# ishine/dmel_codec

Hardware: AMD Instinct MI355X
Metric: audio-sec/sec (encode+decode RTF) @24 kHz batch 32 (higher is better)
Workload: dtype f32; 1 GPU; cfg2: encode+decode, 24000 Hz, 80 mel, 8 FSQ groups [7, 5, 5], WaveNet 20+20 layers, BigVGAN-base, batch 32 x 1 s per GPU; lanes=3, vocoder_streams=1

## Files before the change

### dmel_codec_amd/_lib.py

```python
from __future__ import annotations

import ctypes as C
import os
from typing import Optional, Sequence

import torch

_HERE = os.path.dirname(os.path.abspath(__file__))
LIB_PATH = os.environ.get("DMEL_LIB") or os.path.join(_HERE, "libdmel_hip.so")
_lib: Optional[C.CDLL] = None

i64p = C.POINTER(C.c_int64)
i32p = C.POINTER(C.c_int32)
f32p = C.POINTER(C.c_float)
vp = C.c_void_p
GRAD_READY_FN = C.CFUNCTYPE(None, vp, C.c_int64, C.c_int64)


class BigVGANConfig(C.Structure):
    _fields_ = [
        ("num_mels", C.c_int),
        ("upsample_initial_channel", C.c_int),
        ("num_upsamples", C.c_int),
        ("upsample_rates", C.c_int * 8),
# ... 10 lines not shown


PROTOTYPES = {
    "dmel_last_error": (C.c_char_p, []),
    "dmel_abi_version": (C.c_int, []),
    "dmel_stft_plan_create": (C.c_int, [C.POINTER(vp), C.c_int, C.c_int, C.c_int, C.c_int, C.c_int, C.c_double, C.c_double, vp]),
    "dmel_stft_plan_destroy": (None, [vp]),
    "dmel_mel_basis_host": (C.c_int, [C.c_int, C.c_int, C.c_int, C.c_double, C.c_double, vp]),
    "dmel_stft_plan_mel_basis": (C.c_int, [vp, vp]),
    "dmel_stft_num_frames": (C.c_int64, [vp, C.c_int64]),
    "dmel_stft_logmel_f32": (C.c_int, [vp, vp, C.c_int64, vp, vp, C.c_int, C.c_int64, vp]),
    "dmel_resample_f32": (C.c_int, [vp, vp, vp, C.c_int, C.c_int64, C.c_int64, C.c_int, C.c_int, C.c_int, vp]),
    "dmel_resample_window_f32": (C.c_int, [vp, C.c_int64, C.c_int64, C.c_int64, vp, vp, C.c_int, C.c_int64, C.c_int64, C.c_int64, C.c_int, C.c_int,
                                           C.c_int, vp]),
    "dmel_resample_window_items_f32": (C.c_int, [vp, C.c_int64, C.c_int64, i64p, i64p, vp, C.c_int64, i64p, vp, C.c_int64, i64p, C.c_int, i64p,
                                                 C.c_int, i64p, i64p, i64p, vp, vp]),
    "dmel_pcm_convert_items": (C.c_int, [C.POINTER(vp), i32p, C.POINTER(vp), i32p, i64p, C.c_int, vp, vp]),
    "dmel_pcm_convert_items_ch": (C.c_int, [C.POINTER(vp), i32p, i32p, i32p, C.POINTER(vp), i32p, i32p, i64p, C.c_int, vp, vp]),
    "dmel_stft_f32": (C.c_int, [vp, vp, C.c_int64, vp, vp, vp, C.c_int, C.c_int64, vp]),
    "dmel_stft_window_f32": (C.c_int, [vp, vp, C.c_int64, C.c_int64, C.c_int64, vp, vp, vp, C.c_int, C.c_int64, C.c_int64, C.c_int64, vp]),
    "dmel_stft_window_items_f32": (C.c_int, [vp, vp, C.c_int64, C.c_int64, i64p, i64p, vp, vp, vp, C.c_int, i64p, i64p, i64p, vp, vp]),
    "dmel_aa_snake_f32": (C.c_int, [vp, vp, vp, vp, vp, vp, C.c_int, C.c_int, C.c_int, C.c_int64, vp]),
    "dmel_aa_snake_items_f32": (C.c_int, [vp, vp, vp, vp, vp, vp, C.c_int, C.c_int, C.c_int, C.c_int64, vp, vp]),
    "dmel_aa_snake_backward_f32": (C.c_int, [vp, vp, vp, vp, vp, vp, vp, vp, vp, C.c_int, C.c_int, C.c_int, C.c_int64, vp]),
    "dmel_discriminator_create": (C.c_int, [C.POINTER(vp)]),
    "dmel_discriminator_destroy": (None, [vp]),
    "dmel_discriminator_set_tensor": (C.c_int, [vp, C.c_char_p, vp, C.POINTER(C.c_int64), C.c_int]),
    "dmel_discriminator_finalize": (C.c_int, [vp]),
    "dmel_discriminator_out_frames": (C.c_int64, [vp, C.c_int64]),
    "dmel_discriminator_workspace_bytes": (C.c_size_t, [vp, C.c_int, C.c_int, C.c_int64]),
    "dmel_discriminator_forward": (C.c_int, [vp, vp, vp, C.c_int, C.c_int, C.c_int64, vp, C.c_size_t, vp]),
    "dmel_discriminator_enable_training": (C.c_int, [vp, C.c_int]),
    "dmel_discriminator_set_train_precision": (C.c_int, [vp, C.c_int]),
    "dmel_discriminator_refresh": (C.c_int, [vp, C.c_int, C.POINTER(C.c_char_p), C.POINTER(vp), vp]),
    "dmel_discriminator_train_workspace_bytes": (C.c_size_t, [vp, C.c_int, C.c_int, C.c_int64]),
    "dmel_discriminator_grad_floats": (C.c_int64, [vp]),
    "dmel_discriminator_grad_slot": (C.c_int, [vp, C.c_char_p, C.POINTER(C.c_int64), C.POINTER(C.c_int64)]),
    "dmel_discriminator_forward_train": (C.c_int, [vp, vp, vp, C.c_int, C.c_int, C.c_int64, vp, C.c_size_t, vp]),
    "dmel_discriminator_backward": (C.c_int, [vp, vp, vp, vp, C.c_int, C.c_int, C.c_int64, vp, C.c_size_t, vp]),
    "dmel_convnext_create": (C.c_int, [C.POINTER(vp), C.c_int]),
    "dmel_convnext_destroy": (None, [vp]),
    "dmel_convnext_set_tensor": (C.c_int, [vp, C.c_char_p, vp, C.POINTER(C.c_int64), C.c_int]),
    "dmel_convnext_enable_training": (C.c_int, [vp, C.c_int]),
    "dmel_convnext_set_train_precision": (C.c_int, [vp, C.c_int]),
    "dmel_convnext_finalize": (C.c_int, [vp]),
    "dmel_convnext_workspace_bytes": (C.c_size_t, [vp, C.c_int, C.c_int64]),
# ... 178 lines not shown
```

### dmel_codec_amd/csrc/aa_snake.hip

```cpp
#include "ops.h"
#include "snake_dev.h"

namespace dmel {

constexpr int kSnakeTile = 1024;
constexpr int kSnakeFwdTile = 1008;

typedef float f32x4 __attribute__((ext_vector_type(4)));

template <bool VEC>
__device__ __forceinline__ void aa_snake_row(const float* __restrict__ xr, float* __restrict__ yr, const float* __restrict__ alpha,
                                             const float* __restrict__ beta, const Taps12& tu, const Taps12& td, int logscale, int c, int T,
                                             int first, int nsub, float* xs, float* ve, float* vo) {
  float a = alpha[c], bt = beta ? beta[c] : a;
  if (logscale) {
    bt = beta ? expf(bt) : expf(a);
    a = expf(a);
  }
  const float inv_b = 1.0f / (bt + 1e-9f);
  const int tid = threadIdx.x;
  auto fetch = [&](int t0) {
    const int s = t0 - 8 + 4 * tid;
    if (VEC && s >= 0 && s + 4 <= T) return *reinterpret_cast<const f32x4*>(xr + s);
    f32x4 v;
    v.x = xr[min(max(s, 0), T - 1)];
    v.y = xr[min(max(s + 1, 0), T - 1)];
    v.z = xr[min(max(s + 2, 0), T - 1)];
    v.w = xr[min(max(s + 3, 0), T - 1)];
    return v;
  };
  float aa[8], bb[8];
#pragma unroll
  for (int i = 0; i < 8; ++i) { aa[i] = a; bb[i] = inv_b; }
  f32x4 pre = {0.f, 0.f, 0.f, 0.f};
  if (first < T) pre = fetch(first);
  for (int sub = 0; sub < nsub; ++sub) {
    const int t0 = first + sub * kSnakeFwdTile;
    if (t0 >= T) break;
    const int len = min(kSnakeFwdTile, T - t0);
    if (sub) __syncthreads();
    *reinterpret_cast<f32x4*>(xs + 4 * tid) = pre;
    if (sub + 1 < nsub && t0 + kSnakeFwdTile < T) pre = fetch(t0 + kSnakeFwdTile);
    __syncthreads();
    if (4 * tid < len + 6) {
      float w[12];
      lds_read3_b128(xs + 4 * tid, w);
      float u[8];
#pragma unroll
      for (int i = 0; i < 4; ++i) {
        float ue = 0.f, uo = 0.f;
#pragma unroll
        for (int j = 0; j < 6; ++j) {
          ue = fmaf(tu.f[2 * j + 1], w[i + 7 - j], ue);
          uo = fmaf(tu.f[2 * j], w[i + 8 - j], uo);
        }
        u[2 * i] = ue;
        u[2 * i + 1] = uo;
      }
      snake_n(u, aa, bb);
      *reinterpret_cast<f32x4*>(ve + 4 * tid) = f32x4{u[0], u[2], u[4], u[6]};
      *reinterpret_cast<f32x4*>(vo + 4 * tid) = f32x4{u[1], u[3], u[5], u[7]};
    }
    __syncthreads();
    const int pe = T - t0 + 3;
    if (t0 == 0 || pe < len + 6) {
      if (tid < 3) {
        if (t0 == 0) ve[tid] = vo[tid] = ve[3];
        if (pe + tid < len + 6) ve[pe + tid] = vo[pe + tid] = vo[pe - 1];
      }
      __syncthreads();
    }
    if (4 * tid < len) {
      float e[12], o[12];
      lds_read3_b128(ve + 4 * tid, e);
      lds_read3_b128(vo + 4 * tid, o);
      f32x4 out;
#pragma unroll
      for (int i = 0; i < 4; ++i) {
        float acc = td.f[0] * o[i];
#pragma unroll
        for (int k = 1; k < 6; ++k) {
          acc = fmaf(td.f[2 * k - 1], e[i + k], acc);
          acc = fmaf(td.f[2 * k], o[i + k], acc);
        }
        out[i] = fmaf(td.f[11], e[i + 6], acc);
      }
      float* yp = yr + t0 + 4 * tid;
      if (VEC) {
        *reinterpret_cast<f32x4*>(yp) = out;
      } else {
#pragma unroll
        for (int i = 0; i < 4; ++i)
          if (4 * tid + i < len) yp[i] = out[i];
      }
    }
  }
}

template <bool VEC>
__global__ __launch_bounds__(256) void aa_snake_kernel(const float* __restrict__ x, float* __restrict__ y,
                                                          const float* __restrict__ alpha, const float* __restrict__ beta,
                                                          Taps12 tu, Taps12 td, int logscale, int C, int T, int nsub) {
  __shared__ __attribute__((aligned(16))) float xs[kSnakeFwdTile + 16];
  __shared__ __attribute__((aligned(16))) float ve[kSnakeFwdTile + 16];
  __shared__ __attribute__((aligned(16))) float vo[kSnakeFwdTile + 16];
  const int c = blockIdx.y, b = blockIdx.z;
  const int64_t row = ((int64_t)b * C + c) * T;
  aa_snake_row<VEC>(x + row, y + row, alpha, beta, tu, td, logscale, c, T, blockIdx.x * nsub * kSnakeFwdTile, nsub, xs, ve, vo);
}

__global__ __launch_bounds__(256) void aa_snake_items_kernel(const float* __restrict__ x, float* __restrict__ y,
                                                                const float* __restrict__ alpha, const float* __restrict__ beta,
                                                                Taps12 tu, Taps12 td, int logscale, int C, int T,
                                                                const int64_t* __restrict__ len, int nsub) {
  __shared__ __attribute__((aligned(16))) float xs[kSnakeFwdTile + 16];
  __shared__ __attribute__((aligned(16))) float ve[kSnakeFwdTile + 16];
  __shared__ __attribute__((aligned(16))) float vo[kSnakeFwdTile + 16];
  const int c = blockIdx.y, b = blockIdx.z;
  const int n = (int)min(max(len[b], (int64_t)0), (int64_t)T);
  const int first = blockIdx.x * nsub * kSnakeFwdTile;
  if (first >= n) return;
  const int64_t row = ((int64_t)b * C + c) * T;
  const float* xr = x + row;
  float* yr = y + row;
  const bool vec = n % 4 == 0 && (reinterpret_cast<uintptr_t>(xr) | reinterpret_cast<uintptr_t>(yr)) % 16 == 0;
  if (vec) aa_snake_row<true>(xr, yr, alpha, beta, tu, td, logscale, c, n, first, nsub, xs, ve, vo);
  else aa_snake_row<false>(xr, yr, alpha, beta, tu, td, logscale, c, n, first, nsub, xs, ve, vo);
}

template <bool PARAMS>
__global__ __launch_bounds__(256) void aa_snake_bwd_kernel(const float* __restrict__ x, const float* __restrict__ dy,
                                                            float* dx, const float* __restrict__ alpha,
                                                            const float* __restrict__ beta, float* __restrict__ dalpha,
                                                            float* __restrict__ dbeta, const float* __restrict__ radd, const float* racc,
                                                            Taps12 tu, Taps12 td, int logscale, int C, int T) {
  __shared__ float xs[kSnakeTile + 12];
  __shared__ float dys[kSnakeTile + 12];
  __shared__ float dvs[2 * (kSnakeTile + 6)];
  __shared__ float dxs[kSnakeTile];
  __shared__ float red[2][4];
  const int c = blockIdx.y, b = blockIdx.z, tid = threadIdx.x;
  const int t0 = blockIdx.x * kSnakeTile;
  const int len = min(kSnakeTile, T - t0);
  const float* xr = x + ((int64_t)b * C + c) * T;
  const float* dyr = dy + ((int64_t)b * C + c) * T;
  float* dxr = dx + ((int64_t)b * C + c) * T;
  float a = alpha[c], bt = beta ? beta[c] : a;
  if (logscale) {
    bt = beta ? expf(bt) : expf(a);
    a = expf(a);
// ... 167 lines not shown
    else hipLaunchKernelGGL(aa_snake_kernel<false>, grid, dim3(256), 0, s, x, y, alpha, beta, tu, td, logscale, C, (int)T, nsub);
  }
  DMEL_HIP(hipGetLastError());
  return DMEL_OK;
}

int launch_aa_snake_items(const float* x, float* y, const float* alpha, const float* beta, const float* up_taps_host,
                          const float* down_taps_host, int logscale, int B, int C, int64_t T, const int64_t* len, hipStream_t s) {
  DMEL_CHECK_ARG(x && y && alpha && up_taps_host && down_taps_host && len, "aa_snake_items: NULL argument");
  DMEL_CHECK_ARG(B > 0 && C > 0 && T > 0 && B <= 65535 && C <= 65535 && T < ((int64_t)1 << 30), "aa_snake_items: bad shape");
  Taps12 tu, td;
  for (int i = 0; i < 12; ++i) { tu.f[i] = 2.f * up_taps_host[i]; td.f[i] = down_taps_host[i]; }
  constexpr int nsub = 3;
  constexpr int span = kSnakeFwdTile * nsub;
  dim3 grid((unsigned)((T + span - 1) / span), (unsigned)C, (unsigned)B);
  {
    ProfScope ps("aa_snake", s, 0.0, 8.0 * (double)B * C * (double)T);
    hipLaunchKernelGGL(aa_snake_items_kernel, grid, dim3(256), 0, s, x, y, alpha, beta, tu, td, logscale, C, (int)T, len, nsub);
  }
  DMEL_HIP(hipGetLastError());
  return DMEL_OK;
}

}

extern "C" int dmel_aa_snake_items_f32(const float* x, float* y, const float* alpha, const float* beta, const float* up_filter12_host,
                                       const float* down_filter12_host, int logscale, int B, int C, int64_t T, const int64_t* lengths_dev,
                                       void* stream) {
  return dmel::launch_aa_snake_items(x, y, alpha, beta, up_filter12_host, down_filter12_host, logscale, B, C, T, lengths_dev,
                                     (hipStream_t)stream);
}

extern "C" int dmel_aa_snake_backward_f32(const float* x, const float* dy, float* dx, const float* alpha, const float* beta,
                                          float* dalpha, float* dbeta, const float* up_filter12_host, const float* down_filter12_host,
                                          int logscale, int B, int C, int64_t T, void* stream) {
  return dmel::launch_aa_snake_bwd(x, dy, dx, alpha, beta, dalpha, dbeta, up_filter12_host, down_filter12_host, logscale, B, C, T,
                                   (hipStream_t)stream);
}

extern "C" int dmel_aa_snake_backward_input_f32(const float* x, const float* dy, const float* add , float* dx, const float* alpha,
                                                const float* beta, const float* up_filter12_host, const float* down_filter12_host,
                                                int logscale, int B, int C, int64_t T, void* stream) {
  return dmel::launch_aa_snake_bwd_input(x, dy, dx, add, nullptr, alpha, beta, up_filter12_host, down_filter12_host, logscale, B, C, T,
                                         (hipStream_t)stream);
}

// ... 5 lines not shown
```

### dmel_codec_amd/csrc/modules.hip

```cpp
#include <cmath>
#include <cstdlib>
#include <map>
#include <memory>
#include <mutex>

#include "ops.h"

using namespace dmel;

namespace {

struct HostTensor {
  std::vector<float> v;
  std::vector<int64_t> shape;
  int64_t numel() const { return (int64_t)v.size(); }
};

struct TensorStore {
  std::map<std::string, HostTensor> t;
  int set(const char* key, const float* data, const int64_t* shape, int ndim) {
    DMEL_CHECK_ARG(key && data && shape && ndim >= 0 && ndim <= 4, "set_tensor: bad argument");
    HostTensor h;
    int64_t n = 1;
    for (int i = 0; i < ndim; ++i) { h.shape.push_back(shape[i]); n *= shape[i]; }
// ... 2572 lines not shown
  float* ua = bufs[4];

  {
    ConvRun r = run_1seg(mel, c.num_mels, T, x, c.upsample_initial_channel, T, B);
    r.seg[0].in_len = len_at(0);
    r.precision = prec;
    DMEL_TRY(launch_conv(m->conv_pre, r, st));
  }
  int64_t Tc = T;
  int ch = c.upsample_initial_channel;
  for (int i = 0; i < c.num_upsamples; ++i) {
    const UpStage& us = m->ups[i];
    const int64_t Tn = Tc * us.u;
    DMEL_TRY(launch_up_stage(us, x, xu, B, Tc, prec, st, len_at(i)));
    ch = us.Cout;
    Tc = Tn;
    const int64_t bs = (int64_t)ch * Tc;
    const bool multi = m->multi;
    const int64_t* len = len_at(i + 1);
    if (multi) {
      DMEL_HIP(hipEventRecord(m->ev_fork, st));
      for (int k = 0; k < dmel_bigvgan::kSide; ++k) DMEL_HIP(hipStreamWaitEvent(m->side[k], m->ev_fork, 0));
    }
    for (int j = 0; j < c.num_kernels; ++j) {
      const AmpBlock& ab = m->blocks[(size_t)i * c.num_kernels + j];
      hipStream_t sj = (multi && j > 0) ? m->side[j - 1] : st;
      float *xj = bufs[3 + 3 * j], *uj = bufs[4 + 3 * j], *vj = bufs[5 + 3 * j];
      const float* xin = xu;
      const char* fuse_env = getenv("DMEL_FUSE_SNAKE");
      const bool fuse = fuse_env && fuse_env[0] == '1' && !lengths;
      for (int l = 0; l < 3; ++l) {
        if (l == 0 && multi && j > 0) DMEL_HIP(hipStreamWaitEvent(sj, m->ev_stag[j - 1], 0));
        if (c.resblock_type == 2) {
          ConvRun r2 = run_1seg(uj, ch, Tc, l < 2 ? xj : xs, ch, Tc, B);
          r2.seg[0].in_len = len;
          r2.res = xin; r2.res_bs = bs; r2.res_cs = Tc;
          r2.precision = prec;
          const bool fuse2 = fuse && conv_snake_eligible(ab.c1[l], r2);
          if (!fuse2) DMEL_TRY(act(xin, uj, ab.act[l], ch, Tc, len, sj));
          if (!fuse2 && l == 0 && multi && j + 1 < c.num_kernels) DMEL_HIP(hipEventRecord(m->ev_stag[j], sj));
          if (l == 2) {
            r2.accumulate = j > 0;
            if (j == c.num_kernels - 1) r2.out_div = (float)c.num_kernels;
            if (multi && j > 0) DMEL_HIP(hipStreamWaitEvent(sj, m->ev_chain[j - 1], 0));
          }
          if (fuse2) {
            r2.seg[0].x = xin;
            DMEL_TRY(launch_conv_snake(ab.c1[l], r2, ab.act[l].alpha.as<float>(), ab.act[l].beta.as<float>(), m->taps_up, m->taps_dn, logscale, sj));
            if (l == 0 && multi && j + 1 < c.num_kernels) DMEL_HIP(hipEventRecord(m->ev_stag[j], sj));
          } else {
            DMEL_TRY(launch_conv(ab.c1[l], r2, sj));
          }
          if (l == 2 && multi && j + 1 < c.num_kernels) DMEL_HIP(hipEventRecord(m->ev_chain[j], sj));
          xin = xj;
          continue;
        }
        ConvRun r1 = run_1seg(uj, ch, Tc, vj, ch, Tc, B);
        r1.seg[0].in_len = len;
        r1.precision = prec;
        if (fuse && conv_snake_eligible(ab.c1[l], r1)) {
          r1.seg[0].x = xin;
          DMEL_TRY(launch_conv_snake(ab.c1[l], r1, ab.act[2 * l].alpha.as<float>(), ab.act[2 * l].beta.as<float>(), m->taps_up, m->taps_dn, logscale, sj));
          if (l == 0 && multi && j + 1 < c.num_kernels) DMEL_HIP(hipEventRecord(m->ev_stag[j], sj));
        } else {
          DMEL_TRY(act(xin, uj, ab.act[2 * l], ch, Tc, len, sj));
          if (l == 0 && multi && j + 1 < c.num_kernels) DMEL_HIP(hipEventRecord(m->ev_stag[j], sj));
          DMEL_TRY(launch_conv(ab.c1[l], r1, sj));
        }
        ConvRun r2 = run_1seg(uj, ch, Tc, l < 2 ? xj : xs, ch, Tc, B);
        r2.seg[0].in_len = len;
        r2.res = xin; r2.res_bs = bs; r2.res_cs = Tc;
        r2.precision = prec;
        const bool fuse2 = fuse && conv_snake_eligible(ab.c2[l], r2);
        if (!fuse2) DMEL_TRY(act(vj, uj, ab.act[2 * l + 1], ch, Tc, len, sj));
        if (l == 2) {
          r2.accumulate = j > 0;
          if (j == c.num_kernels - 1) r2.out_div = (float)c.num_kernels;
          if (multi && j > 0) DMEL_HIP(hipStreamWaitEvent(sj, m->ev_chain[j - 1], 0));
        }
        if (fuse2) {
          r2.seg[0].x = vj;
          DMEL_TRY(launch_conv_snake(ab.c2[l], r2, ab.act[2 * l + 1].alpha.as<float>(), ab.act[2 * l + 1].beta.as<float>(), m->taps_up, m->taps_dn, logscale, sj));
        } else {
          DMEL_TRY(launch_conv(ab.c2[l], r2, sj));
        }
        if (l == 2 && multi && j + 1 < c.num_kernels) DMEL_HIP(hipEventRecord(m->ev_chain[j], sj));
        xin = xj;
      }
    }
    if (multi) {
      for (int k = 0; k < dmel_bigvgan::kSide && k + 1 < c.num_kernels; ++k) {
        DMEL_HIP(hipEventRecord(m->ev_join[k], m->side[k]));
        DMEL_HIP(hipStreamWaitEvent(st, m->ev_join[k], 0));
      }
    }
    std::swap(x, xs);
  }
  const int64_t* len_out = len_at(c.num_upsamples);
  DMEL_TRY(act(x, ua, m->act_post, ch, Tc, len_out, st));
  return launch_conv_post(ua, audio, m->post_w.as<float>(), m->post_bias, c.use_tanh_at_final ? ACT_TANH : ACT_CLAMP1, B, ch, 7,
                          Tc, st, len_out);
}

extern "C" int dmel_bigvgan_forward(const dmel_bigvgan* m, const float* mel, float* audio, int B, int64_t T, void* workspace,
                                    size_t workspace_bytes, void* stream) {
  return bigvgan_forward_impl(m, mel, nullptr, audio, B, T, workspace, workspace_bytes, stream);
}

extern "C" int dmel_bigvgan_forward_items(const dmel_bigvgan* m, const float* mel, const int64_t* lengths_dev, float* audio, int B, int64_t T,
                                          void* workspace, size_t workspace_bytes, void* stream) {
  DMEL_CHECK_ARG(lengths_dev, "bigvgan_forward_items: NULL lengths");
  return bigvgan_forward_impl(m, mel, lengths_dev, audio, B, T, workspace, workspace_bytes, stream);
}

extern "C" int dmel_bigvgan_enable_input_grad(dmel_bigvgan* m, int on) {
  DMEL_CHECK_ARG(m, "bigvgan_enable_input_grad: NULL handle");
  if (!m->ready) { set_error("bigvgan_enable_input_grad: handle not finalized"); return DMEL_EMISSING; }
  const dmel_bigvgan_config& c = m->cfg;
  if (!on) {
    m->input_grad = false;
    m->conv_preT = PackedConv();
// ... 243 lines not shown
```

### dmel_codec_amd/csrc/ops.h

```cpp
#pragma once
#include "conv.h"

namespace dmel {

struct FsqConst {
  int n_levels;
  int levels[4], half_width[4], basis[4];
  float half_l[4], offset[4], shift[4];
  int prebound;
  int strict;
};

int make_fsq_const(FsqConst& k, const int* levels, int n, int prebound);
int launch_fsq_encode(const float* z, const float* w_in, const float* b_in, int32_t* ids, float* prequant,
                      const FsqConst& k, int B, int G, int C, int64_t T4, hipStream_t s, const int64_t* len = nullptr);
int launch_fsq_decode(const int32_t* ids, const float* w_out, const float* b_out, float* z, const FsqConst& k, int B,
                      int G, int C, int64_t T4, hipStream_t s, const int64_t* len = nullptr);
int launch_fsq_backward(const float* x, const float* dout, const float* w_in, const float* b_in, const float* w_out, float* dx,
                        float* dw_in, float* db_in, float* dw_out, float* db_out, float* scratch, const FsqConst& k, int B, int G, int C,
                        int64_t T4, hipStream_t s);
int launch_dwconv_ln(const float* x, float* y, const float* dw_w, const float* dw_b, const float* ln_w, const float* ln_b,
                     int N, int C, int64_t T, hipStream_t s, float* h0 = nullptr, const int64_t* len = nullptr, int len_div = 1);
int launch_conv_post(const float* x, float* y, const float* w_dev, float bias, int act, int B, int C, int K, int64_t T,
                     hipStream_t s, const int64_t* len = nullptr);
// ... 18 lines not shown
};
int launch_wavenet_fused(const WaveNetFused& f, const float* x, float* y, const int64_t* in_len, const int64_t* out_len, int len_div, int N,
                         int64_t T, hipStream_t st);
constexpr int kStreamMaxL = 32;
int launch_wavenet_stream(const WaveNetFused& f, const float* x, float* hist, float* skip, float* y, const int64_t* out_len, int len_div,
                          int N, int64_t cap, const int64_t* prev, const int64_t* next, hipStream_t st);
constexpr int kStreamRowInts(int L) { return 2 * (L + 1) + 1; }
int launch_wavenet_stream_items(const WaveNetFused& f, const float* x, float* hist, float* skip, float* y, const int64_t* out_len, int len_div,
                                int N, int64_t cap, const int64_t* prev, const int64_t* next, int32_t* tab_dev, hipStream_t st);
int launch_shift_lengths(const int64_t* len, int64_t shift, int64_t* out, int n, hipStream_t st);
int launch_copy_windows(const float* src, float* dst, int N, int C, int64_t cap, const int32_t* tab, int stride, int i_shift, int i_end,
                        int len_div, int64_t max_cols, int64_t cols_total, hipStream_t st);
int launch_shift_lengths_items(const int64_t* len, const int32_t* tab, int stride, int i_shift, int64_t* out, int n, hipStream_t st);
struct LenScales {
  static constexpr int kMax = 9;
  int64_t v[kMax];
};
int launch_length_tables(const int64_t* len, int64_t* tab, int n, int64_t T, int stages, const LenScales& scale, hipStream_t st);
int launch_stage_lengths(const int64_t* len, int64_t* tab, int n, int64_t T, int stages, int down, hipStream_t st);
int launch_aa_snake(const float* x, float* y, const float* alpha, const float* beta, const float* up_taps_host,
                    const float* down_taps_host, int logscale, int B, int C, int64_t T, hipStream_t s);
int launch_aa_snake_items(const float* x, float* y, const float* alpha, const float* beta, const float* up_taps_host,
                          const float* down_taps_host, int logscale, int B, int C, int64_t T, const int64_t* len, hipStream_t s);
int launch_aa_snake_bwd_input(const float* x, const float* dy, float* dx, const float* radd, const float* racc, const float* alpha,
                              const float* beta, const float* up_taps_host, const float* down_taps_host, int logscale, int B, int C,
                              int64_t T, hipStream_t s);

bool conv_snake_eligible(const PackedConv& pc, const ConvRun& r);
int launch_conv_snake(const PackedConv& pc, const ConvRun& r, const float* alpha, const float* beta, const float* up_taps_host,
                      const float* down_taps_host, int logscale, hipStream_t stream);

bool conv_pc_eligible(const PackedConv& pc, const ConvRun& r, bool any_size = false);
int launch_conv_pc(const PackedConv& pc, const ConvRun& r, hipStream_t stream);

int launch_gate_fwd(const float* pre, float* z, int N, int C, int64_t T, hipStream_t s);
int launch_gate_bwd(const float* dz, const float* pre, float* dpre, int N, int C, int64_t T, hipStream_t s);
int launch_resskip_fwd(const float* x, const float* o, float* xn, float* skipsum, int first, int N, int C, int64_t T, hipStream_t s);
int launch_resskip_bwd(const float* gx, const float* gs, float* go, float* gxs, int N, int C, int64_t T, hipStream_t s);
int launch_silu_fwd(const float* u, float* y, int64_t total, hipStream_t s);
int launch_silu_bwd(const float* g, const float* u, float* du, int64_t total, hipStream_t s);
int launch_scale(const float* x, float* y, float k, int64_t total, hipStream_t s);
int launch_gelu_fwd(const float* u, float* g, int64_t total, hipStream_t s);
int launch_gelu_bwd(const float* dg, const float* u, float* du, int64_t total, hipStream_t s);
int launch_layerscale_res_fwd(const float* x, const float* v, const float* gamma, float* y, int N, int C, int64_t T, hipStream_t s);
int launch_layerscale_bwd(const float* dy, const float* v, const float* gamma, float* dv, float* dgamma, int N, int C, int64_t T,
                          hipStream_t s);
// ... 13 lines not shown
```

### include/dmel_hip.h

```cpp
#ifndef DMEL_HIP_H
#define DMEL_HIP_H

#include <stddef.h>
#include <stdint.h>

#ifdef __cplusplus
extern "C" {
#endif

#define DMEL_OK 0
#define DMEL_EINVAL (-1)
#define DMEL_EUNSUPPORTED (-2)
#define DMEL_EMISSING (-3)

#define DMEL_PRECISION_FP32 0
#define DMEL_PRECISION_BF16 1
#define DMEL_PRECISION_FP32_MFMA 2
#define DMEL_PRECISION_FP32_F16X2 3
#define DMEL_PRECISION_FP32_BF16X3 4

const char* dmel_last_error(void);
int dmel_abi_version(void);

typedef struct dmel_stft_plan dmel_stft_plan;
// ... 35 lines not shown
                                   int64_t bank_arena_floats, const int64_t* rates, int n_rates, const int64_t* rate_index, int B,
                                   const int64_t* o0, const int64_t* n_out, const int64_t* total_length, int64_t* table_scratch,
                                   void* stream);

#define DMEL_SAMPLE_F32 0
#define DMEL_SAMPLE_S16 1
#define DMEL_SAMPLE_ULAW 8
#define DMEL_SAMPLE_ALAW 9
int dmel_pcm_convert_items(const void* const* src, const int32_t* src_fmt, void* const* dst, const int32_t* dst_fmt, const int64_t* n,
                           int B, void* table_scratch, void* stream);
#define DMEL_MAX_CHANNELS 8
int dmel_pcm_convert_items_ch(const void* const* src, const int32_t* src_fmt, const int32_t* src_ch, const int32_t* src_pick,
                              void* const* dst, const int32_t* dst_fmt, const int32_t* dst_ch, const int64_t* n, int B,
                              void* table_scratch, void* stream);

int dmel_collate_peak_f32(const float* const* clips_dev, const int64_t* lengths_dev, const int32_t* order_dev , float* audios,
                          int32_t* audio_lengths, uint32_t* peaks_scratch, int B, int64_t Lmax, float peak, void* stream);

int dmel_aa_snake_f32(const float* x, float* y, const float* alpha, const float* beta, const float* up_filter12_host,
                      const float* down_filter12_host, int logscale, int B, int C, int64_t T, void* stream);
int dmel_aa_snake_items_f32(const float* x, float* y, const float* alpha, const float* beta, const float* up_filter12_host,
                            const float* down_filter12_host, int logscale, int B, int C, int64_t T, const int64_t* lengths_dev,
                            void* stream);
int dmel_aa_snake_backward_f32(const float* x, const float* dy, float* dx, const float* alpha, const float* beta ,
                               float* dalpha, float* dbeta , const float* up_filter12_host,
                               const float* down_filter12_host, int logscale, int B, int C, int64_t T, void* stream);

int dmel_aa_snake_backward_input_f32(const float* x, const float* dy, const float* add , float* dx, const float* alpha,
                                     const float* beta , const float* up_filter12_host, const float* down_filter12_host,
                                     int logscale, int B, int C, int64_t T, void* stream);


typedef struct dmel_wavenet dmel_wavenet;
int dmel_wavenet_create(dmel_wavenet** m, int input_channels , int output_channels ,
                        int residual_channels, int residual_layers, int dilation_cycle, int condition_channels );
void dmel_wavenet_destroy(dmel_wavenet* m);
int dmel_wavenet_set_precision(dmel_wavenet* m, int precision);
int dmel_wavenet_set_tensor(dmel_wavenet* m, const char* key, const float* data_host, const int64_t* shape, int ndim);
int dmel_wavenet_finalize(dmel_wavenet* m);
size_t dmel_wavenet_workspace_bytes(const dmel_wavenet* m, int N, int64_t T);
int dmel_wavenet_forward(const dmel_wavenet* m, const float* x, const float* condition, float* y, int N, int64_t T,
                         const int64_t* in_lengths, const int64_t* out_lengths, int group_repeat,
                         void* workspace, size_t workspace_bytes, void* stream);

int dmel_wavenet_enable_training(dmel_wavenet* m, int on);
int dmel_wavenet_set_train_precision(dmel_wavenet* m, int precision);
// ... 236 lines not shown
```

Before: 2717 audio-sec/sec.

## Fuse BigVGAN first-layer snake activations across resblocks and fuse post snake into conv_post

Adds a kernel that reads the upsampled input once and computes the anti-aliased snake activation for all three resblock branches, sharing the upsampling filter pass. The separate per-branch first activations are skipped when this path is on. A second kernel fuses the final snake activation with the 7-tap output convolution and tanh/clamp, so the activated intermediate is never written to global memory. Both paths are on by default and can be disabled with environment variables. They use more shared memory and serialize the three branches inside one block, and the post kernel loops over all channels per block, which may limit parallelism.

```diff
diff --git a/dmel_codec_amd/_lib.py b/dmel_codec_amd/_lib.py
--- a/dmel_codec_amd/_lib.py
+++ b/dmel_codec_amd/_lib.py
@@ -56,6 +56,10 @@
     "dmel_stft_window_items_f32": (C.c_int, [vp, vp, C.c_int64, C.c_int64, i64p, i64p, vp, vp, vp, C.c_int, i64p, i64p, i64p, vp, vp]),
     "dmel_aa_snake_f32": (C.c_int, [vp, vp, vp, vp, vp, vp, C.c_int, C.c_int, C.c_int, C.c_int64, vp]),
     "dmel_aa_snake_items_f32": (C.c_int, [vp, vp, vp, vp, vp, vp, C.c_int, C.c_int, C.c_int, C.c_int64, vp, vp]),
+    "dmel_aa_snake3_forward": (C.c_int, [vp] * 12 + [C.c_int, C.c_int, C.c_int, C.c_int64, vp]),
+    "dmel_aa_snake3_forward_items": (C.c_int, [vp] * 12 + [C.c_int, C.c_int, C.c_int, C.c_int64, vp, vp]),
+    "dmel_snake_post_forward": (C.c_int, [vp, vp, vp, vp, vp, C.c_int, vp, C.c_float, C.c_int, vp, C.c_int, C.c_int, C.c_int, C.c_int64, vp]),
+    "dmel_snake_post_forward_items": (C.c_int, [vp, vp, vp, vp, vp, C.c_int, vp, C.c_float, C.c_int, vp, C.c_int, C.c_int, C.c_int, C.c_int64, vp, vp]),
     "dmel_aa_snake_backward_f32": (C.c_int, [vp, vp, vp, vp, vp, vp, vp, vp, vp, C.c_int, C.c_int, C.c_int, C.c_int64, vp]),
     "dmel_discriminator_create": (C.c_int, [C.POINTER(vp)]),
     "dmel_discriminator_destroy": (None, [vp]),
diff --git a/dmel_codec_amd/csrc/aa_snake.hip b/dmel_codec_amd/csrc/aa_snake.hip
--- a/dmel_codec_amd/csrc/aa_snake.hip
+++ b/dmel_codec_amd/csrc/aa_snake.hip
@@ -7,59 +7,90 @@
 constexpr int kSnakeFwdTile = 1008;
 
 typedef float f32x4 __attribute__((ext_vector_type(4)));
+
+template <bool VEC>
+__device__ __forceinline__ f32x4 snake_fetch4(const float* __restrict__ xr, int T, int t0, int tid) {
+  const int s = t0 - 8 + 4 * tid;
+  if (VEC && s >= 0 && s + 4 <= T) return *reinterpret_cast<const f32x4*>(xr + s);
+  f32x4 v;
+  v.x = xr[min(max(s, 0), T - 1)];
+  v.y = xr[min(max(s + 1, 0), T - 1)];
+  v.z = xr[min(max(s + 2, 0), T - 1)];
+  v.w = xr[min(max(s + 3, 0), T - 1)];
+  return v;
+}
+__device__ __forceinline__ void snake_up4(const float* xs, int tid, const Taps12& tu, float (&u)[8]) {
+  float w[12];
+  lds_read3_b128(xs + 4 * tid, w);
+#pragma unroll
+  for (int i = 0; i < 4; ++i) {
+    float ue = 0.f, uo = 0.f;
+#pragma unroll
+    for (int j = 0; j < 6; ++j) {
+      ue = fmaf(tu.f[2 * j + 1], w[i + 7 - j], ue);
+      uo = fmaf(tu.f[2 * j], w[i + 8 - j], uo);
+    }
+    u[2 * i] = ue;
+    u[2 * i + 1] = uo;
+  }
+}
+__device__ __forceinline__ void snake_store4(float (&u)[8], float a, float inv_b, float* ve, float* vo, int tid) {
+  float aa[8], bb[8];
+#pragma unroll
+  for (int i = 0; i < 8; ++i) { aa[i] = a; bb[i] = inv_b; }
+  snake_n(u, aa, bb);
+  *reinterpret_cast<f32x4*>(ve + 4 * tid) = f32x4{u[0], u[2], u[4], u[6]};
+  *reinterpret_cast<f32x4*>(vo + 4 * tid) = f32x4{u[1], u[3], u[5], u[7]};
+}
+__device__ __forceinline__ f32x4 snake_down4(const float* ve, const float* vo, int tid, const Taps12& td) {
+  float e[12], o[12];
+  lds_read3_b128(ve + 4 * tid, e);
+  lds_read3_b128(vo + 4 * tid, o);
+  f32x4 out;
+#pragma unroll
+  for (int i = 0; i < 4; ++i) {
+    float acc = td.f[0] * o[i];
+#pragma unroll
+    for (int k = 1; k < 6; ++k) {
+      acc = fmaf(td.f[2 * k - 1], e[i + k], acc);
+      acc = fmaf(td.f[2 * k], o[i + k], acc);
+    }
+    out[i] = fmaf(td.f[11], e[i + 6], acc);
+  }
+  return out;
+}
+__device__ __forceinline__ void snake_params(const float* __restrict__ alpha, const float* __restrict__ beta, int logscale, int c, float& a,
+                                             float& inv_b) {
+  a = alpha[c];
+  float bt = beta ? beta[c] : a;
+  if (logscale) {
+    bt = beta ? expf(bt) : expf(a);
+    a = expf(a);
+  }
+  inv_b = 1.0f / (bt + 1e-9f);
+}
 
 template <bool VEC>
 __device__ __forceinline__ void aa_snake_row(const float* __restrict__ xr, float* __restrict__ yr, const float* __restrict__ alpha,
                                              const float* __restrict__ beta, const Taps12& tu, const Taps12& td, int logscale, int c, int T,
                                              int first, int nsub, float* xs, float* ve, float* vo) {
-  float a = alpha[c], bt = beta ? beta[c] : a;
-  if (logscale) {
-    bt = beta ? expf(bt) : expf(a);
-    a = expf(a);
-  }
-  const float inv_b = 1.0f / (bt + 1e-9f);
+  float a, inv_b;
+  snake_params(alpha, beta, logscale, c, a, inv_b);
   const int tid = threadIdx.x;
-  auto fetch = [&](int t0) {
-    const int s = t0 - 8 + 4 * tid;
-    if (VEC && s >= 0 && s + 4 <= T) return *reinterpret_cast<const f32x4*>(xr + s);
-    f32x4 v;
-    v.x = xr[min(max(s, 0), T - 1)];
-    v.y = xr[min(max(s + 1, 0), T - 1)];
-    v.z = xr[min(max(s + 2, 0), T - 1)];
-    v.w = xr[min(max(s + 3, 0), T - 1)];
-    return v;
-  };
-  float aa[8], bb[8];
-#pragma unroll
-  for (int i = 0; i < 8; ++i) { aa[i] = a; bb[i] = inv_b; }
   f32x4 pre = {0.f, 0.f, 0.f, 0.f};
-  if (first < T) pre = fetch(first);
+  if (first < T) pre = snake_fetch4<VEC>(xr, T, first, tid);
   for (int sub = 0; sub < nsub; ++sub) {
     const int t0 = first + sub * kSnakeFwdTile;
     if (t0 >= T) break;
     const int len = min(kSnakeFwdTile, T - t0);
     if (sub) __syncthreads();
     *reinterpret_cast<f32x4*>(xs + 4 * tid) = pre;
-    if (sub + 1 < nsub && t0 + kSnakeFwdTile < T) pre = fetch(t0 + kSnakeFwdTile);
+    if (sub + 1 < nsub && t0 + kSnakeFwdTile < T) pre = snake_fetch4<VEC>(xr, T, t0 + kSnakeFwdTile, tid);
     __syncthreads();
     if (4 * tid < len + 6) {
-      float w[12];
-      lds_read3_b128(xs + 4 * tid, w);
       float u[8];
-#pragma unroll
-      for (int i = 0; i < 4; ++i) {
-        float ue = 0.f, uo = 0.f;
-#pragma unroll
-        for (int j = 0; j < 6; ++j) {
-          ue = fmaf(tu.f[2 * j + 1], w[i + 7 - j], ue);
-          uo = fmaf(tu.f[2 * j], w[i + 8 - j], uo);
-        }
-        u[2 * i] = ue;
-        u[2 * i + 1] = uo;
-      }
-      snake_n(u, aa, bb);
-      *reinterpret_cast<f32x4*>(ve + 4 * tid) = f32x4{u[0], u[2], u[4], u[6]};
-      *reinterpret_cast<f32x4*>(vo + 4 * tid) = f32x4{u[1], u[3], u[5], u[7]};
+      snake_up4(xs, tid, tu, u);
+      snake_store4(u, a, inv_b, ve, vo, tid);
     }
     __syncthreads();
     const int pe = T - t0 + 3;
@@ -71,20 +102,7 @@
       __syncthreads();
     }
     if (4 * tid < len) {
-      float e[12], o[12];
-      lds_read3_b128(ve + 4 * tid, e);
-      lds_read3_b128(vo + 4 * tid, o);
-      f32x4 out;
-#pragma unroll
-      for (int i = 0; i < 4; ++i) {
-        float acc = td.f[0] * o[i];
-#pragma unroll
-        for (int k = 1; k < 6; ++k) {
-          acc = fmaf(td.f[2 * k - 1], e[i + k], acc);
-          acc = fmaf(td.f[2 * k], o[i + k], acc);
-        }
-        out[i] = fmaf(td.f[11], e[i + 6], acc);
-      }
+      const f32x4 out = snake_down4(ve, vo, tid, td);
       float* yp = yr + t0 + 4 * tid;
       if (VEC) {
         *reinterpret_cast<f32x4*>(yp) = out;
@@ -126,6 +144,189 @@
   const bool vec = n % 4 == 0 && (reinterpret_cast<uintptr_t>(xr) | reinterpret_cast<uintptr_t>(yr)) % 16 == 0;
   if (vec) aa_snake_row<true>(xr, yr, alpha, beta, tu, td, logscale, c, n, first, nsub, xs, ve, vo);
   else aa_snake_row<false>(xr, yr, alpha, beta, tu, td, logscale, c, n, first, nsub, xs, ve, vo);
+}
+
+struct Snake3 {
+  float* y[3];
+  const float* alpha[3];
+  const float* beta[3];
+};
+
+template <bool VEC>
+__device__ __forceinline__ void aa_snake3_row(const float* __restrict__ xr, int64_t row, const Snake3& p, const Taps12& tu, const Taps12& td,
+                                              int logscale, int c, int T, int first, int nsub, int yvec, float* xs, float* planes) {
+  float a[3], inv_b[3];
+#pragma unroll
+  for (int k = 0; k < 3; ++k) snake_params(p.alpha[k], p.beta[k], logscale, c, a[k], inv_b[k]);
+  const int tid = threadIdx.x;
+  f32x4 pre = {0.f, 0.f, 0.f, 0.f};
+  if (first < T) pre = snake_fetch4<VEC>(xr, T, first, tid);
+  int par = 0;
+  for (int sub = 0; sub < nsub; ++sub) {
+    const int t0 = first + sub * kSnakeFwdTile;
+    if (t0 >= T) break;
+    const int len = min(kSnakeFwdTile, T - t0);
+    *reinterpret_cast<f32x4*>(xs + 4 * tid) = pre;
+    if (sub + 1 < nsub && t0 + kSnakeFwdTile < T) pre = snake_fetch4<VEC>(xr, T, t0 + kSnakeFwdTile, tid);
+    __syncthreads();
+    const bool pairs = 4 * tid < len + 6;
+    float u[8];
+    if (pairs) snake_up4(xs, tid, tu, u);
+    const int pe = T - t0 + 3;
+#pragma unroll
+    for (int k = 0; k < 3; ++k) {
+      float* ve = planes + par * 2 * (kSnakeFwdTile + 16);
+      float* vo = ve + (kSnakeFwdTile + 16);
+      par ^= 1;
+      if (pairs) {
+        float v[8];
+#pragma unroll
+        for (int i = 0; i < 8; ++i) v[i] = u[i];
+        snake_store4(v, a[k], inv_b[k], ve, vo, tid);
+      }
+      __syncthreads();
+      if (t0 == 0 || pe < len + 6) {
+        if (tid < 3) {
+          if (t0 == 0) ve[tid] = vo[tid] = ve[3];
+          if (pe + tid < len + 6) ve[pe + tid] = vo[pe + tid] = vo[pe - 1];
+        }
+        __syncthreads();
+      }
+      if (4 * tid < len) {
+        const f32x4 out = snake_down4(ve, vo, tid, td);
+        float* yp = p.y[k] + row + t0 + 4 * tid;
+        if (VEC && ((yvec >> k) & 1)) {
+          *reinterpret_cast<f32x4*>(yp) = out;
+        } else {
+#pragma unroll
+          for (int i = 0; i < 4; ++i)
+            if (4 * tid + i < len) yp[i] = out[i];
+        }
+      }
+    }
+  }
+}
+
+template <bool VEC>
+__global__ __launch_bounds__(256) void aa_snake3_kernel(const float* __restrict__ x, Snake3 p, Taps12 tu, Taps12 td, int logscale, int C, int T,
+                                                           int nsub, int yvec) {
+  __shared__ __attribute__((aligned(16))) float xs[kSnakeFwdTile + 16];
+  __shared__ __attribute__((aligned(16))) float planes[4 * (kSnakeFwdTile + 16)];
+  const int c = blockIdx.y, b = blockIdx.z;
+  const int64_t row = ((int64_t)b * C + c) * T;
+  aa_snake3_row<VEC>(x + row, row, p, tu, td, logscale, c, T, blockIdx.x * nsub * kSnakeFwdTile, nsub, yvec, xs, planes);
+}
+
+__global__ __launch_bounds__(256) void aa_snake3_items_kernel(const float* __restrict__ x, Snake3 p, Taps12 tu, Taps12 td, int logscale, int C,
+                                                                 int T, const int64_t* __restrict__ len, int nsub) {
+  __shared__ __attribute__((aligned(16))) float xs[kSnakeFwdTile + 16];
+  __shared__ __attribute__((aligned(16))) float planes[4 * (kSnakeFwdTile + 16)];
+  const int c = blockIdx.y, b = blockIdx.z;
+  const int n = (int)min(max(len[b], (int64_t)0), (int64_t)T);
+  const int first = blockIdx.x * nsub * kSnakeFwdTile;
+  if (first >= n) return;
+  const int64_t row = ((int64_t)b * C + c) * T;
+  const float* xr = x + row;
+  int yvec = 0;
+#pragma unroll
+  for (int k = 0; k < 3; ++k) yvec |= (int)(reinterpret_cast<uintptr_t>(p.y[k] + row) % 16 == 0) << k;
+  const bool vec = n % 4 == 0 && reinterpret_cast<uintptr_t>(xr) % 16 == 0;
+  if (vec) aa_snake3_row<true>(xr, row, p, tu, td, logscale, c, n, first, nsub, yvec, xs, planes);
+  else aa_snake3_row<false>(xr, row, p, tu, td, logscale, c, n, first, nsub, 0, xs, planes);
+}
+
+template <int KT>
+__global__ __launch_bounds__(256) void snake_post_kernel(const float* __restrict__ x, float* __restrict__ y, const float* __restrict__ alpha,
+                                                            const float* __restrict__ beta, Taps12 tu, Taps12 td, int logscale,
+                                                            const float* __restrict__ w, float bias, int act, int C, int K, int T,
+                                                            const int64_t* __restrict__ len) {
+  __shared__ __attribute__((aligned(16))) float xs[kSnakeFwdTile + 16];
+  __shared__ __attribute__((aligned(16))) float ve[kSnakeFwdTile + 16];
+  __shared__ __attribute__((aligned(16))) float vo[kSnakeFwdTile + 16];
+  __shared__ __attribute__((aligned(16))) float as[kSnakeFwdTile + 16];
+  const int tid = threadIdx.x, b = blockIdx.y;
+  const int pad = (KT ? KT : K) / 2, H = (pad + 3) & ~3, W = kSnakeFwdTile - 2 * H;
+  const int first = blockIdx.x * W;
+  const int n = len ? (int)min(max(len[b], (int64_t)0), (int64_t)T) : T;
+  float* yb = y + (int64_t)b * T;
+  if (first >= n) {
+    for (int t = first + tid; t < min(first + W, T); t += 256) yb[t] = 0.f;
+    return;
+  }
+  const int t0 = first - H;
+  const int alen = min(kSnakeFwdTile, n - t0);
+  const float* xr = x + (int64_t)b * C * T;
+  const bool vec = T % 4 == 0 && reinterpret_cast<uintptr_t>(x) % 16 == 0;
+  float acc[4];
+#pragma unroll
+  for (int e = 0; e < 4; ++e) acc[e] = bias;
+  f32x4 pre = vec ? snake_fetch4<true>(xr, n, t0, tid) : snake_fetch4<false>(xr, n, t0, tid);
+  const int pz = 3 - t0;
+  const int pe = n - t0 + 3;
+  for (int c = 0; c < C; ++c) {
+    float a, inv_b;
+    snake_params(alpha, beta, logscale, c, a, inv_b);
+    *reinterpret_cast<f32x4*>(xs + 4 * tid) = pre;
+    if (c + 1 < C) {
+      xr += T;
+      pre = vec ? snake_fetch4<true>(xr, n, t0, tid) : snake_fetch4<false>(xr, n, t0, tid);
+    }
+    __syncthreads();
+    if (4 * tid < alen + 6) {
+      float u[8];
+      snake_up4(xs, tid, tu, u);
+      snake_store4(u, a, inv_b, ve, vo, tid);
+    }
+    __syncthreads();
+    if (t0 <= 0 || pe < alen + 6) {
+      if (tid < 3) {
+        if (t0 <= 0) ve[pz - 1 - tid] = vo[pz - 1 - tid] = ve[pz];
+        if (pe + tid < alen + 6) ve[pe + tid] = vo[pe + tid] = vo[pe - 1];
+      }
+      __syncthreads();
+    }
+    if (4 * tid < kSnakeFwdTile) {
+      f32x4 out = {0.f, 0.f, 0.f, 0.f};
+      if (4 * tid < alen) out = snake_down4(ve, vo, tid, td);
+#pragma unroll
+      for (int i = 0; i < 4; ++i) {
+        const int t = t0 + 4 * tid + i;
+        if (t < 0 || t >= n) out[i] = 0.f;
+      }
+      *reinterpret_cast<f32x4*>(as + 4 * tid) = out;
+    }
+    __syncthreads();
+    if (4 * tid < W) {
+      const float* wc = w + c * (KT ? KT : K);
+      if (KT == 7) {
+        float v[12];
+        lds_read3_b128(as + 4 * tid, v);
+#pragma unroll
+        for (int k = 0; k < 7; ++k) {
+          const float wv = wc[k];
+#pragma unroll
+          for (int e = 0; e < 4; ++e) acc[e] = fmaf(wv, v[e + 1 + k], acc[e]);
+        }
+      } else {
+        const float* ap = as + 4 * tid + (H - pad);
+        for (int k = 0; k < K; ++k) {
+          const float wv = wc[k];
+#pragma unroll
+          for (int e = 0; e < 4; ++e) acc[e] = fmaf(wv, ap[e + k], acc[e]);
+        }
+      }
+    }
+  }
+  if (4 * tid < W) {
+#pragma unroll
+    for (int e = 0; e < 4; ++e) {
+      const int t = first + 4 * tid + e;
+      if (t < T) {
+        const float v = act == 2 ? tanhf(acc[e]) : (act == 3 ? fminf(fmaxf(acc[e], -1.f), 1.f) : acc[e]);
+        yb[t] = t < n ? v : 0.f;
+      }
+    }
+  }
 }
 
 template <bool PARAMS>
@@ -339,6 +540,94 @@
   return DMEL_OK;
 }
 
+int launch_aa_snake3(const float* x, float* const y[3], const float* const alpha[3], const float* const beta[3], const float* up_taps_host,
+                     const float* down_taps_host, int logscale, int B, int C, int64_t T, const int64_t* len, hipStream_t s) {
+  DMEL_CHECK_ARG(x && y && alpha && beta && up_taps_host && down_taps_host, "aa_snake3: NULL argument");
+  DMEL_CHECK_ARG(y[0] && y[1] && y[2] && alpha[0] && alpha[1] && alpha[2], "aa_snake3: NULL output or alpha");
+  DMEL_CHECK_ARG(y[0] != y[1] && y[0] != y[2] && y[1] != y[2] && x != y[0] && x != y[1] && x != y[2], "aa_snake3: x and the outputs must be distinct");
+  DMEL_CHECK_ARG(B > 0 && C > 0 && T > 0 && B <= 65535 && C <= 65535 && T < ((int64_t)1 << 30), "aa_snake3: bad shape");
+  Taps12 tu, td;
+  for (int i = 0; i < 12; ++i) { tu.f[i] = 2.f * up_taps_host[i]; td.f[i] = down_taps_host[i]; }
+  Snake3 p;
+  int yvec = 0;
+  for (int k = 0; k < 3; ++k) {
+    p.y[k] = y[k]; p.alpha[k] = alpha[k]; p.beta[k] = beta[k];
+    yvec |= (int)(reinterpret_cast<uintptr_t>(y[k]) % 16 == 0) << k;
+  }
+  constexpr int nsub = 3;
+  constexpr int span = kSnakeFwdTile * nsub;
+  dim3 grid((unsigned)((T + span - 1) / span), (unsigned)C, (unsigned)B);
+  const bool vec = T % 4 == 0 && reinterpret_cast<uintptr_t>(x) % 16 == 0;
+  {
+    ProfScope ps("aa_snake", s, 0.0, 16.0 * (double)B * C * (double)T);
+    if (len) hipLaunchKernelGGL(aa_snake3_items_kernel, grid, dim3(256), 0, s, x, p, tu, td, logscale, C, (int)T, len, nsub);
+    else if (vec) hipLaunchKernelGGL(aa_snake3_kernel<true>, grid, dim3(256), 0, s, x, p, tu, td, logscale, C, (int)T, nsub, yvec);
+    else hipLaunchKernelGGL(aa_snake3_kernel<false>, grid, dim3(256), 0, s, x, p, tu, td, logscale, C, (int)T, nsub, 0);
+  }
+  DMEL_HIP(hipGetLastError());
+  return DMEL_OK;
+}
+
+constexpr int kPostMaxPad = 128;
+int launch_snake_post(const float* x, float* y, const float* alpha, const float* beta, const float* up_taps_host, const float* down_taps_host,
+                      int logscale, const float* w_dev, float bias, int act, int B, int C, int K, int64_t T, const int64_t* len, hipStream_t s) {
+  DMEL_CHECK_ARG(x && y && alpha && up_taps_host && down_taps_host && w_dev, "snake_post: NULL argument");
+  DMEL_CHECK_ARG(B > 0 && B <= 65535 && C > 0 && K > 0 && (K % 2) == 1 && T > 0 && T < ((int64_t)1 << 30), "snake_post: bad shape");
+  DMEL_CHECK_ARG((size_t)C * K * sizeof(float) <= 48 * 1024, "snake_post: weight table too large");
+  DMEL_CHECK_ARG(K / 2 <= kPostMaxPad, "snake_post: more than %d taps", 2 * kPostMaxPad + 1);
+  Taps12 tu, td;
+  for (int i = 0; i < 12; ++i) { tu.f[i] = 2.f * up_taps_host[i]; td.f[i] = down_taps_host[i]; }
+  const int W = kSnakeFwdTile - 2 * ((K / 2 + 3) & ~3);
+  dim3 grid((unsigned)((T + W - 1) / W), (unsigned)B);
+  {
+    ProfScope ps("small", s, 0.0, 4.0 * B * (double)T * (C + 1));
+    if (K == 7) hipLaunchKernelGGL(snake_post_kernel<7>, grid, dim3(256), 0, s, x, y, alpha, beta, tu, td, logscale, w_dev, bias, act, C, K, (int)T, len);
+    else hipLaunchKernelGGL(snake_post_kernel<0>, grid, dim3(256), 0, s, x, y, alpha, beta, tu, td, logscale, w_dev, bias, act, C, K, (int)T, len);
+  }
+  DMEL_HIP(hipGetLastError());
+  return DMEL_OK;
+}
+
+}
+
+extern "C" int dmel_aa_snake3_forward(const float* x, float* y0, float* y1, float* y2, const float* alpha0, const float* beta0,
+                                      const float* alpha1, const float* beta1, const float* alpha2, const float* beta2,
+                                      const float* up_filter12_host, const float* down_filter12_host, int logscale, int B, int C, int64_t T,
+                                      void* stream) {
+  float* const y[3] = {y0, y1, y2};
+  const float* const al[3] = {alpha0, alpha1, alpha2};
+  const float* const be[3] = {beta0, beta1, beta2};
+  return dmel::launch_aa_snake3(x, y, al, be, up_filter12_host, down_filter12_host, logscale, B, C, T, nullptr, (hipStream_t)stream);
+}
+
+extern "C" int dmel_aa_snake3_forward_items(const float* x, float* y0, float* y1, float* y2, const float* alpha0, const float* beta0,
+                                            const float* alpha1, const float* beta1, const float* alpha2, const float* beta2,
+                                            const float* up_filter12_host, const float* down_filter12_host, int logscale, int B, int C,
+                                            int64_t T, const int64_t* lengths_dev, void* stream) {
+  DMEL_CHECK_ARG(lengths_dev, "aa_snake3_forward_items: NULL lengths");
+  float* const y[3] = {y0, y1, y2};
+  const float* const al[3] = {alpha0, alpha1, alpha2};
+  const float* const be[3] = {beta0, beta1, beta2};
+  return dmel::launch_aa_snake3(x, y, al, be, up_filter12_host, down_filter12_host, logscale, B, C, T, lengths_dev, (hipStream_t)stream);
+}
+
+static int snake_post_entry(const float* x, const float* alpha, const float* beta, const float* up, const float* down, int logscale,
+                            const float* w_dev, float bias, int act, float* y, int B, int C, int K, int64_t T, const int64_t* len, void* stream) {
+  DMEL_CHECK_ARG(act == 0 || act == 2 || act == 3, "snake_post: act must be 0 (none), 2 (tanh) or 3 (clamp to [-1, 1])");
+  return dmel::launch_snake_post(x, y, alpha, beta, up, down, logscale, w_dev, bias, act, B, C, K, T, len, (hipStream_t)stream);
+}
+
+extern "C" int dmel_snake_post_forward(const float* x, const float* alpha, const float* beta, const float* up_filter12_host,
+                                       const float* down_filter12_host, int logscale, const float* w_dev, float bias, int act, float* y, int B,
+                                       int C, int K, int64_t T, void* stream) {
+  return snake_post_entry(x, alpha, beta, up_filter12_host, down_filter12_host, logscale, w_dev, bias, act, y, B, C, K, T, nullptr, stream);
+}
+
+extern "C" int dmel_snake_post_forward_items(const float* x, const float* alpha, const float* beta, const float* up_filter12_host,
+                                             const float* down_filter12_host, int logscale, const float* w_dev, float bias, int act, float* y,
+                                             int B, int C, int K, int64_t T, const int64_t* lengths_dev, void* stream) {
+  DMEL_CHECK_ARG(lengths_dev, "snake_post_forward_items: NULL lengths");
+  return snake_post_entry(x, alpha, beta, up_filter12_host, down_filter12_host, logscale, w_dev, bias, act, y, B, C, K, T, lengths_dev, stream);
 }
 
 extern "C" int dmel_aa_snake_items_f32(const float* x, float* y, const float* alpha, const float* beta, const float* up_filter12_host,
diff --git a/dmel_codec_amd/csrc/modules.hip b/dmel_codec_amd/csrc/modules.hip
--- a/dmel_codec_amd/csrc/modules.hip
+++ b/dmel_codec_amd/csrc/modules.hip
@@ -2618,13 +2618,25 @@
       DMEL_HIP(hipEventRecord(m->ev_fork, st));
       for (int k = 0; k < dmel_bigvgan::kSide; ++k) DMEL_HIP(hipStreamWaitEvent(m->side[k], m->ev_fork, 0));
     }
+    const char* fuse_env = getenv("DMEL_FUSE_SNAKE");
+    const bool fuse = fuse_env && fuse_env[0] == '1' && !lengths;
+    const char* head_env = getenv("DMEL_SNAKE_HEAD3");
+    const bool head3 = !multi && !fuse && c.num_kernels == 3 && !(head_env && head_env[0] == '0');
+    if (head3) {
+      float* const hy[3] = {bufs[4], bufs[7], bufs[10]};
+      const float *ha[3], *hb[3];
+      for (int j = 0; j < 3; ++j) {
+        const SnakeP& p = m->blocks[(size_t)i * 3 + j].act[0];
+        ha[j] = p.alpha.as<float>();
+        hb[j] = p.beta.as<float>();
+      }
+      DMEL_TRY(launch_aa_snake3(xu, hy, ha, hb, m->taps_up, m->taps_dn, logscale, B, ch, Tc, len, st));
+    }
     for (int j = 0; j < c.num_kernels; ++j) {
       const AmpBlock& ab = m->blocks[(size_t)i * c.num_kernels + j];
       hipStream_t sj = (multi && j > 0) ? m->side[j - 1] : st;
       float *xj = bufs[3 + 3 * j], *uj = bufs[4 + 3 * j], *vj = bufs[5 + 3 * j];
       const float* xin = xu;
-      const char* fuse_env = getenv("DMEL_FUSE_SNAKE");
-      const bool fuse = fuse_env && fuse_env[0] == '1' && !lengths;
       for (int l = 0; l < 3; ++l) {
         if (l == 0 && multi && j > 0) DMEL_HIP(hipStreamWaitEvent(sj, m->ev_stag[j - 1], 0));
         if (c.resblock_type == 2) {
@@ -2633,7 +2645,7 @@
           r2.res = xin; r2.res_bs = bs; r2.res_cs = Tc;
           r2.precision = prec;
           const bool fuse2 = fuse && conv_snake_eligible(ab.c1[l], r2);
-          if (!fuse2) DMEL_TRY(act(xin, uj, ab.act[l], ch, Tc, len, sj));
+          if (!fuse2 && !(head3 && l == 0)) DMEL_TRY(act(xin, uj, ab.act[l], ch, Tc, len, sj));
           if (!fuse2 && l == 0 && multi && j + 1 < c.num_kernels) DMEL_HIP(hipEventRecord(m->ev_stag[j], sj));
           if (l == 2) {
             r2.accumulate = j > 0;
@@ -2659,7 +2671,7 @@
           DMEL_TRY(launch_conv_snake(ab.c1[l], r1, ab.act[2 * l].alpha.as<float>(), ab.act[2 * l].beta.as<float>(), m->taps_up, m->taps_dn, logscale, sj));
           if (l == 0 && multi && j + 1 < c.num_kernels) DMEL_HIP(hipEventRecord(m->ev_stag[j], sj));
         } else {
-          DMEL_TRY(act(xin, uj, ab.act[2 * l], ch, Tc, len, sj));
+          if (!(head3 && l == 0)) DMEL_TRY(act(xin, uj, ab.act[2 * l], ch, Tc, len, sj));
           if (l == 0 && multi && j + 1 < c.num_kernels) DMEL_HIP(hipEventRecord(m->ev_stag[j], sj));
           DMEL_TRY(launch_conv(ab.c1[l], r1, sj));
         }
@@ -2693,6 +2705,10 @@
     std::swap(x, xs);
   }
   const int64_t* len_out = len_at(c.num_upsamples);
+  const char* post_env = getenv("DMEL_POST_FUSED");
+  if (!(post_env && post_env[0] == '0'))
+    return launch_snake_post(x, audio, m->act_post.alpha.as<float>(), m->act_post.beta.as<float>(), m->taps_up, m->taps_dn, logscale,
+                             m->post_w.as<float>(), m->post_bias, c.use_tanh_at_final ? ACT_TANH : ACT_CLAMP1, B, ch, 7, Tc, len_out, st);
   DMEL_TRY(act(x, ua, m->act_post, ch, Tc, len_out, st));
   return launch_conv_post(ua, audio, m->post_w.as<float>(), m->post_bias, c.use_tanh_at_final ? ACT_TANH : ACT_CLAMP1, B, ch, 7,
                           Tc, st, len_out);
diff --git a/dmel_codec_amd/csrc/ops.h b/dmel_codec_amd/csrc/ops.h
--- a/dmel_codec_amd/csrc/ops.h
+++ b/dmel_codec_amd/csrc/ops.h
@@ -64,6 +64,10 @@
                     const float* down_taps_host, int logscale, int B, int C, int64_t T, hipStream_t s);
 int launch_aa_snake_items(const float* x, float* y, const float* alpha, const float* beta, const float* up_taps_host,
                           const float* down_taps_host, int logscale, int B, int C, int64_t T, const int64_t* len, hipStream_t s);
+int launch_aa_snake3(const float* x, float* const y[3], const float* const alpha[3], const float* const beta[3], const float* up_taps_host,
+                     const float* down_taps_host, int logscale, int B, int C, int64_t T, const int64_t* len, hipStream_t s);
+int launch_snake_post(const float* x, float* y, const float* alpha, const float* beta, const float* up_taps_host, const float* down_taps_host,
+                      int logscale, const float* w_dev, float bias, int act, int B, int C, int K, int64_t T, const int64_t* len, hipStream_t s);
 int launch_aa_snake_bwd_input(const float* x, const float* dy, float* dx, const float* radd, const float* racc, const float* alpha,
                               const float* beta, const float* up_taps_host, const float* down_taps_host, int logscale, int B, int C,
                               int64_t T, hipStream_t s);
diff --git a/include/dmel_hip.h b/include/dmel_hip.h
--- a/include/dmel_hip.h
+++ b/include/dmel_hip.h
@@ -81,6 +81,19 @@
 int dmel_aa_snake_items_f32(const float* x, float* y, const float* alpha, const float* beta, const float* up_filter12_host,
                             const float* down_filter12_host, int logscale, int B, int C, int64_t T, const int64_t* lengths_dev,
                             void* stream);
+int dmel_aa_snake3_forward(const float* x, float* y0, float* y1, float* y2, const float* alpha0, const float* beta0, const float* alpha1,
+                           const float* beta1, const float* alpha2, const float* beta2, const float* up_filter12_host,
+                           const float* down_filter12_host, int logscale, int B, int C, int64_t T, void* stream);
+int dmel_aa_snake3_forward_items(const float* x, float* y0, float* y1, float* y2, const float* alpha0, const float* beta0,
+                                 const float* alpha1, const float* beta1, const float* alpha2, const float* beta2,
+                                 const float* up_filter12_host, const float* down_filter12_host, int logscale, int B, int C, int64_t T,
+                                 const int64_t* lengths_dev, void* stream);
+int dmel_snake_post_forward(const float* x, const float* alpha, const float* beta, const float* up_filter12_host,
+                            const float* down_filter12_host, int logscale, const float* w_dev, float bias, int act, float* y, int B, int C,
+                            int K, int64_t T, void* stream);
+int dmel_snake_post_forward_items(const float* x, const float* alpha, const float* beta, const float* up_filter12_host,
+                                  const float* down_filter12_host, int logscale, const float* w_dev, float bias, int act, float* y, int B,
+                                  int C, int K, int64_t T, const int64_t* lengths_dev, void* stream);
 int dmel_aa_snake_backward_f32(const float* x, const float* dy, float* dx, const float* alpha, const float* beta ,
                                float* dalpha, float* dbeta , const float* up_filter12_host,
                                const float* down_filter12_host, int logscale, int B, int C, int64_t T, void* stream);
```

Result: faster. 2744 audio-sec/sec (median of 6 runs) (+1.0%).
